# multimodallearning/DG-TTA

Hardware: AMD Instinct MI355X
Metric: TTA-epochs/sec per GPU on 128^3 patch; Dice delta vs reference (higher is better)
Workload: dtype fp16

## Files before the change

### dg_tta_amd/csrc/common.h

```cpp
#pragma once
#include <hip/hip_runtime.h>
#include <hip/hip_bf16.h>
#include <hip/hip_fp16.h>
#include <stdint.h>
#include <stdio.h>
#include <stdarg.h>

#include "../../include/dgtta.h"

#define WAVE 64

#include <atomic>

void dgtta_set_error(const char *fmt, ...);

struct DgttaSwitches {
  int conv_rows, conv_s2, dgrad_s2_allcls, wgrad_tr, wgrad_tr8, wgrad_s2_onepass, convt_wgrad_onepass;
  int convt_gemm, rows_order, in_nt, wgrad_upw, wgrad_xcd, in_gstats, softdice16, conv_ring, wgrad_ring, ha_mfma, wgrad_f32_split, feature_head_mfma, headwarp_mfma, wgrad_flat, wgrad_reduce_taps;
};
const DgttaSwitches &dgtta_switches();

struct DynLdsOnce {
  std::atomic<unsigned long long> mask{0};
};
static inline hipError_t ensure_dyn_lds(DynLdsOnce &o, const void *fn, int bytes) {
  int dev = 0;
  (void)hipGetDevice(&dev);
  const unsigned long long bit = 1ull << (dev & 63);
  if (o.mask.load(std::memory_order_acquire) & bit) return hipSuccess;
  const hipError_t e = hipFuncSetAttribute(fn, hipFuncAttributeMaxDynamicSharedMemorySize, bytes);
  if (e == hipSuccess) o.mask.fetch_or(bit, std::memory_order_release);
  return e;
}

struct RowsGstCtx {
  const void *y;
  long long ldy;
  const float *mr, *gamma, *beta;
  float slope;
  double *out;
  int produced;
// ... 180 lines not shown
```

### dg_tta_amd/csrc/conv_mfma.hip

```cpp
#include "conv_common.h"
#include <stdlib.h>
#include <type_traits>

namespace {

template <typename T, int MBW, int MBH, int MBD, int S, int NB, int KSPC, int NW = 4, bool AC = false>
__global__ __launch_bounds__(NW * 64) void conv3_mfma_kernel(const T *__restrict__ x, View xv, const T *__restrict__ w,
                                                         ConvClasses cs, const float *__restrict__ bias,
                                                         T *__restrict__ y, View yv, int Cin, int Cout, int CinP,
                                                         int CoutP, int tilesW, int tilesH, int tilesD,
                                                         double *__restrict__ stats, int ntaps_src) {
  const int cls = blockIdx.z;
  x += cs.xoff[cls];
  if (!AC) y += cs.yoff[cls];
  const Taps &taps = cs.taps[cls];
  const int accumulate = cs.acc[cls];
  const int Di = xv.D, Hi = xv.H, Wi = xv.W, Do = yv.D, Ho = yv.H, Wo = yv.W;
  typedef ConvCfg<T, MBW, MBH, MBD, S, NB, KSPC> Cfg;
  typedef typename Cfg::G G;
  constexpr int EPV = Cfg::EPV, NG = Cfg::NG, CK = Cfg::CK, NC = Cfg::NC, NV = G::NV, MPW = G::MB / NW, NT = NW * 64;
  extern __shared__ __attribute__((aligned(16))) unsigned char smem[];
  uint4 *sA = reinterpret_cast<uint4 *>(smem);
  uint4 *sB = reinterpret_cast<uint4 *>(smem + Cfg::A_BYTES);

// ... 288 lines not shown
    }
    if (blockIdx.x == 0 && blockIdx.y == 0 && tid == 0) reinterpret_cast<long long *>(stats)[0] = tiles_per_b;
  }
}

template <typename T, int MBW, int MBH, int MBD, int S, int NB, int KSPC, int NW = 4, bool AC = false>
int launch_conv(const ConvLaunch &L, const ConvClasses &cs) {
  typedef ConvCfg<T, MBW, MBH, MBD, S, NB, KSPC> Cfg;
  typedef typename Cfg::G G;
  auto kern = conv3_mfma_kernel<T, MBW, MBH, MBD, S, NB, KSPC, NW, AC>;
  static DynLdsOnce lds_once;
  DG_REQUIRE(ensure_dyn_lds(lds_once, reinterpret_cast<const void *>(kern), (int)Cfg::LDS_BYTES) == hipSuccess,
             DGTTA_ERR_LAUNCH, "conv3_mfma: cannot raise the dynamic LDS limit to %zu", (size_t)Cfg::LDS_BYTES);
  const int tW = cdiv(L.yv.W, G::TW), tH = cdiv(L.yv.H, G::TH), tD = cdiv(L.yv.D, G::TD);
  const int64_t tiles = (int64_t)tW * tH * tD * L.B;
  DG_REQUIRE(tiles < (1ll << 31), DGTTA_ERR_UNSUPPORTED, "conv3_mfma: too many tiles");
  dim3 grid((unsigned)tiles, (unsigned)cdiv(L.CoutP, Cfg::NC), AC ? 1u : (unsigned)cs.n);
  hipLaunchKernelGGL(kern, grid, dim3(NW * 64), Cfg::LDS_BYTES, L.st, (const T *)L.x, L.xv, (const T *)L.w, cs, L.bias, (T *)L.y,
                     L.yv, L.Cin, L.Cout, L.CinP, L.CoutP, tW, tH, tD, L.stats, L.ntaps_src);
  DG_CHECK_LAUNCH(AC ? "conv3_mfma_kernel<all classes>" : "conv3_mfma_kernel");
  return DGTTA_OK;
}

template <typename T>
int dispatch_conv_classes(const ConvLaunch &L, const ConvClasses &cs, int stride) {
  const View &yv = L.yv;
  const bool ring_only = L.xkh || L.dry;
  const long long vox = (long long)yv.D * yv.H * yv.W * L.B;
  if (ring_only && stride != 1) return DGTTA_ERR_UNSUPPORTED;
  if (stride == 0) {
    if (yv.W >= 32) return launch_conv<T, 32, 4, 4, 0, 1, 1, 8>(L, cs);
    if (yv.W >= 16) return launch_conv<T, 16, 4, 4, 0, 1, 1, 8>(L, cs);
    if (vox <= 4096) return launch_conv<T, 8, 2, 2, 0, 1, 1>(L, cs);
    return launch_conv<T, 8, 2, 8, 0, 1, 1, 8>(L, cs);
  }
  if (stride == 1 && sizeof(T) == 2 && yv.W >= 32 && cs.n == 1 && cs.acc[0] == 0 && cs.kseg == 0 && cs.xoff[0] == 0 &&
      cs.yoff[0] == 0) {
    const int rows = dgtta_switches().conv_rows;
    const int is_f16 = (int)std::is_same<T, f16_t>::value;
    bool all_taps = true;
    for (int t = 0; t < 27; ++t) all_taps = all_taps && cs.taps[0].wt[t] >= 0;
    const bool vec_out = L.Cout % 8 == 0 && ((uintptr_t)L.y & 15) == 0 && yv.sw % 8 == 0 && yv.sh % 8 == 0 &&
                         yv.sd % 8 == 0 && yv.sb % 8 == 0;
    const long long njobs = (long long)cdiv(yv.W, 32) * cdiv(yv.H, 8) * cdiv(yv.D, 4) * cdiv(L.CoutP, 32) * L.B;
    if (all_taps && vec_out && ((L.Cin == 32 && L.CinP == 32) || (L.Cin == 64 && L.CinP == 64)) &&
        (njobs >= 512 || dgtta_switches().conv_ring == '1') && dgtta_switches().conv_ring != '0' && rows != '1') {
      const int rc = conv3_ring_launch(L, cs.taps[0], conv3_mfma_max_tiles(yv.D, yv.H, yv.W), is_f16);
      if (rc != DGTTA_ERR_UNSUPPORTED || ring_only) return rc;
    }
    if (ring_only) return DGTTA_ERR_UNSUPPORTED;
    if (all_taps && vec_out && (njobs >= 256 || rows == '1') && rows != '0') return conv3_rows_launch(L, cs.taps[0], is_f16);
  }
  if (ring_only) return DGTTA_ERR_UNSUPPORTED;
  if (stride == 1) {
    if (yv.W >= 32) return launch_conv<T, 32, 4, 4, 1, 1, 1, 8>(L, cs);
    const bool k2 = L.CinP % (4 * Elem<T>::EPV) == 0;
    if (yv.W >= 16) return launch_conv<T, 16, 4, 4, 1, 1, 1, 8>(L, cs);
    if (vox <= 4096 && k2) return launch_conv<T, 8, 2, 2, 1, 1, 2>(L, cs);
    if (vox <= 4096) return launch_conv<T, 8, 2, 2, 1, 1, 1>(L, cs);
    return launch_conv<T, 8, 2, 8, 1, 1, 1, 8>(L, cs);
  }
  if (stride == 2) {
    if (dgtta_switches().conv_s2 == '4') {
      if (yv.W >= 16) return launch_conv<T, 16, 2, 4, 2, 1, 1>(L, cs);
      return launch_conv<T, 8, 2, 4, 2, 1, 1>(L, cs);
    }
    if (dgtta_switches().conv_s2 != '1' && yv.W >= 32 && L.CoutP % 64 == 0) return launch_conv<T, 32, 4, 2, 2, 2, 1, 8>(L, cs);
    if (yv.W >= 32) return launch_conv<T, 32, 4, 2, 2, 1, 1, 8>(L, cs);
    if (yv.W >= 16) return launch_conv<T, 16, 2, 4, 2, 1, 1, 8>(L, cs);
    return launch_conv<T, 8, 2, 4, 2, 1, 1, 8>(L, cs);
  }
  return DGTTA_ERR_UNSUPPORTED;
}

template <typename T>
int dispatch_conv(const ConvLaunch &L, const Taps &taps, int stride, int accumulate) {
  return dispatch_conv_classes<T>(L, single_class(taps, accumulate), stride);
}

template <typename T>
int dgrad_s2_allcls(const ConvLaunch &L, const ConvClasses &cs) {
  if (L.yv.W >= 32) return launch_conv<T, 32, 4, 2, 1, 1, 1, 8, true>(L, cs);
  if (L.yv.W >= 16) return launch_conv<T, 16, 2, 4, 1, 1, 1, 8, true>(L, cs);
  return launch_conv<T, 8, 2, 4, 1, 1, 1, 8, true>(L, cs);
}

template <typename T>
__global__ void conva_pack_kernel(const float *__restrict__ w, T *__restrict__ imgF, T *__restrict__ imgB, int Cin, int Cout,
                                  int CinP, int CoutP, int ntaps) {
  constexpr int EPV = Elem<T>::EPV;
  const int CoutN = (CoutP + 31) / 32 * 32, CinN = (CinP + 31) / 32 * 32;
// ... 11 lines not shown
    }
  }
}

}

int64_t conv3_mfma_max_tiles(int Do, int Ho, int Wo) {
  const int shapes[6][3] = {{4, 4, 32}, {4, 8, 16}, {2, 8, 8}, {8, 8, 8}, {4, 4, 16}, {4, 8, 8}};
  int64_t best = 0;
  for (auto &t : shapes) {
    int64_t n = (int64_t)cdiv(Do, t[0]) * cdiv(Ho, t[1]) * cdiv(Wo, t[2]);
    best = n > best ? n : best;
  }
  return best;
}

int conv3_fwd_mfma(const ConvProblem &P, Src x, const void *w_kmajor, int mirror, const float *bias, Dst y, double *stats,
                   RowsGstCtx *gst) {
  const int stride = P.sd, dtype = P.dtype;
  if ((x.kh || P.dry) && (stride != 1 || dtype == DGTTA_F32)) return DGTTA_ERR_UNSUPPORTED;
  const int Do = P.Do(), Ho = P.Ho(), Wo = P.Wo();
  const ConvLaunch L{x.p, dense_view(P.B, P.Di, P.Hi, P.Wi, x.ld), w_kmajor, bias, y.p, dense_view(P.B, Do, Ho, Wo, y.ld), P.B, P.Cin,
                     P.Cout, P.CinP, P.CoutP, stats, 27, P.st, gst, x.kh, P.dry};
  if (stride == 2 && !mirror && dtype != DGTTA_F32 && dgtta_switches().conv_s2 != '1' && dgtta_switches().conv_s2 != '4') {
    const int rc = conv3_s2_regs(L, conv3_mfma_max_tiles(Do, Ho, Wo), dtype);
    if (rc != DGTTA_ERR_UNSUPPORTED) return rc;
  }
  if (!dtype_ok(dtype) || !operand_ok(epv_of(dtype), x.p, x.kh ? 2 * x.ld : x.ld, P.Cin, P.CinP)) return DGTTA_ERR_UNSUPPORTED;
  DISPATCH_T(dtype, return dispatch_conv<T>(L, identity_taps(mirror), stride, 0));
}

int conv3_dgrad_s2_mfma(const ConvProblem &P, Src dy, const void *w_kmajor, Dst dx, int accumulate) {
  if (!dtype_ok(P.dtype) || !operand_ok(epv_of(P.dtype), dy.p, dy.ld, P.Cout, P.CoutP)) return DGTTA_ERR_UNSUPPORTED;
  View yv;
  const ConvClasses cs = dgrad_parity_classes(P, dx.ld, accumulate, &yv);
  const ConvProblem G = dgrad_as_fwd(P);
  const ConvLaunch L{dy.p, dense_view(P.B, P.Do(), P.Ho(), P.Wo(), dy.ld), w_kmajor, nullptr, dx.p, yv, G.B, G.Cin, G.Cout, G.CinP, G.CoutP,
                     nullptr, 27, P.st};
  const bool allcls = dgtta_switches().dgrad_s2_allcls != '0' && P.CinP % 8 == 0;
  DISPATCH_T(P.dtype, return allcls ? dgrad_s2_allcls<T>(L, cs) : dispatch_conv_classes<T>(L, cs, 1));
}

size_t convT_packed_bytes(int CinP, int CoutP, int dtype) {
  return (size_t)8 * (CinP * n32(CoutP) + CoutP * n32(CinP)) * esize(dtype);
}
size_t conv_image_bytes(int CinP, int CoutP, int dtype) {
  return (size_t)27 * (CinP * n32(CoutP) + CoutP * n32(CinP)) * esize(dtype);
// ... 86 lines not shown
```

### dg_tta_amd/csrc/conv_wgrad.hip

```cpp
#include "conv_wgrad_common.h"

WgradPlan wgrad_plan(int B, int Cin, int Cout, int D, int H, int W, int ncls, int tileW, int tileH) {
  WgradPlan p;
  p.tW = cdiv(W, tileW);
  p.tH = cdiv(H, tileH);
  p.cibs = cdiv(Cin, 32);
  p.cobs = cdiv(Cout, 32);
  const int64_t base = (int64_t)B * p.tW * p.tH * p.cibs * p.cobs * ncls;
  int want = (int)cdiv64(512, base > 0 ? base : 1);
  int maxsplit = D / 4 > 0 ? D / 4 : 1;
  p.nsd = want < 1 ? 1 : (want > maxsplit ? maxsplit : want);
  p.DR = cdiv(D, p.nsd);
  p.nsd = cdiv(D, p.DR);
  p.units = (int64_t)B * p.tW * p.tH * p.nsd;
  return p;
}

size_t conv3_wgrad_mfma_ws_bytes(int B, int Cin, int Cout, int D, int H, int W) {
  WgradPlan p1 = wgrad_plan(B, Cin, Cout, D, H, W, 1, 32, WT::TH), p8 = wgrad_plan(B, Cin, Cout, D, H, W, 8, 32, WT::TH),
            p2 = wgrad_plan(B, Cin, Cout, D, H, W, 1, WT2::TWO, WT2::TH);
  const size_t a = wgrad_slab_bytes(p1, 1), b = wgrad_slab_bytes(p8, 8), c = wgrad_slab_bytes(p2, 1);
  return a > b ? (a > c ? a : c) : (b > c ? b : c);
}

static int units_per_workgroup(int64_t units, int64_t gy, int slots) {
  const int sw = dgtta_switches().wgrad_upw;
  if (sw == '1') return 1;
  if (sw >= '2' && sw <= '4') return (int)(units < sw - '0' ? units : sw - '0');
  int64_t u = units * gy / slots;
  if (u > 4) u = 4;
  if (u > units) u = units;
  return u < 1 ? 1 : (int)u;
}

int wgrad_launch_classes(const WgradLaunch &L, const WgradOut &out, const WgradClasses &wc, const RealTaps &reals) {
  if (!dtype_ok(L.dtype)) return DGTTA_ERR_UNSUPPORTED;
  const int esz = (int)esize(L.dtype), EPV = 16 / esz;
  const View &xv = L.xv, &yv = L.yv;
  if (L.Cout % EPV || xv.sw % EPV || yv.sw % EPV || ((uintptr_t)L.x & 15) || ((uintptr_t)L.dy & 15) ||
      xv.sw < (L.xkh ? 32 : (L.Cin + EPV - 1) / EPV * EPV))
    return DGTTA_ERR_UNSUPPORTED;
  for (int c = 0; c < wc.n; ++c)
    if ((wc.xoff[c] * (long long)esz) % 16 || (wc.yoff[c] * (long long)esz) % 16) return DGTTA_ERR_UNSUPPORTED;
  const DgttaSwitches &sw = dgtta_switches();
  if (L.xkh && (esz != 2 || sw.wgrad_tr == '0' || sw.wgrad_ring == '0')) return DGTTA_ERR_UNSUPPORTED;
  WgradPlan p = wgrad_plan(L.B, L.Cin, L.Cout, yv.D, yv.H, yv.W, wc.n, 32, WT::TH);
  if (L.ws_bytes < wgrad_slab_bytes(p, wc.n) || p.units >= (1ll << 31) || p.cibs * p.cobs > 65535) return DGTTA_ERR_UNSUPPORTED;
  int64_t nslab = p.units;
  int rc = DGTTA_OK;
  if (esz == 2 && sw.wgrad_tr != '0') {
    const bool plain = wc.n == 1 && wc.mask[0] == 0x7ffffffu && wc.xoff[0] == 0 && wc.yoff[0] == 0;
    int64_t g = 0;
    if (plain && !L.xkh && !L.split_leg && sw.wgrad_flat != '0') {
// ... 12 lines not shown
      const int upw = units_per_workgroup(p.units, (int64_t)p.cibs * ((p.cobs + 1) / 2), 256);
      nslab = cdiv64(p.units, upw);
      rc = conv3_wgrad_tr8_launch(L, p, upw, nslab);
    } else {
      const int upw = plain ? units_per_workgroup(p.units, (int64_t)p.cibs * p.cobs, 512) : 1;
      nslab = cdiv64(p.units, upw);
      rc = conv3_wgrad_tr_launch(L, p, wc, plain, upw, nslab);
    }
  } else {
    rc = conv3_wgrad_mfma_launch(L, p, wc);
  }
  if (rc != DGTTA_OK) return rc;
  return wgrad_reduce_launch(L, out, p, wc.n, nslab, reals);
}

static int wgrad_conv(const ConvProblem &P, const WgradLaunch &L, const WgradOut &out) {
  RealTaps reals;
  if (P.sd == 1) return wgrad_launch_classes(L, out, wgrad_single_class(0x7ffffffu, identity_taps(0), &reals), reals);
  if (L.xkh) return DGTTA_ERR_UNSUPPORTED;
  if (L.dtype != DGTTA_F32) {
    const int one = dgtta_switches().wgrad_s2_onepass;
    WgradPlan p = wgrad_plan(L.B, L.Cin, L.Cout, L.yv.D, L.yv.H, L.yv.W, 1, WT2::TWO, WT2::TH);
    if (wgrad_onepass_ok(L, p) && one != '0') {
      const int rc = conv3_wgrad_s2_launch(L, p, p.cobs % 2 == 0 && L.Cout % 64 == 0 && one != '1');
      if (rc != DGTTA_OK) return rc;
      reals.t[0] = identity_taps(0);
      return wgrad_reduce_launch(L, out, p, 1, p.units, reals);
    }
  }
  WgradLaunch C = L;
  const WgradClasses wc = wgrad_parity_classes(P, (int)L.xv.sw, &reals, &C.xv);
  return wgrad_launch_classes(C, out, wc, reals);
}

namespace {
__device__ __forceinline__ void split3(float v, bf16_t &a0, bf16_t &a1, bf16_t &a2) {
  a0 = f32_to_bf16(v);
  const float r1 = v - bf16_to_f32(a0);
  a1 = f32_to_bf16(r1);
  const float r2 = r1 - bf16_to_f32(a1);
  a2 = f32_to_bf16(r2);
}

__global__ __launch_bounds__(256) void split3_bf16_kernel(const float *__restrict__ x, int ld, int C, int lds, int64_t n,
                                                        bf16_t *__restrict__ p0, bf16_t *__restrict__ p1,
                                                        bf16_t *__restrict__ p2) {
  const int groups = lds >> 3;
  const int64_t total = n * groups;
  const bool vec = (ld & 3) == 0 && (C & 7) == 0 && (((uintptr_t)x) & 15) == 0;
  for (int64_t i = (int64_t)blockIdx.x * blockDim.x + threadIdx.x; i < total; i += (int64_t)gridDim.x * blockDim.x) {
// ... 120 lines not shown
```

### dg_tta_amd/csrc/conv_wgrad_common.h

```cpp
#pragma once
#include "conv_common.h"
#include <functional>
#include <type_traits>

namespace dgconv {
struct WgradClasses {
  int n;
  unsigned mask[8];
  long long xoff[8], yoff[8];
};
struct RealTaps {
  Taps t[8];
};
struct WgradPlan {
  int tW, tH, nsd, DR, cibs, cobs;
  int64_t units;
};

struct WgradLaunch {
  const void *x;
  View xv;
  const void *dy;
  View yv;
  int B, Cin, Cout, dtype;
// ... 19 lines not shown
  return (size_t)ncls * p.units * p.cibs * p.cobs * 27 * 1024 * sizeof(float);
}
static inline bool wgrad_onepass_ok(const WgradLaunch &L, const WgradPlan &p) {
  return L.Cout % 8 == 0 && L.xv.sw % 8 == 0 && L.yv.sw % 8 == 0 && !((uintptr_t)L.x & 15) && !((uintptr_t)L.dy & 15) &&
         L.xv.sw >= (L.Cin + 7) / 8 * 8 && L.ws_bytes >= wgrad_slab_bytes(p, 1) && p.units < (1ll << 31) && p.cibs * p.cobs <= 65535;
}

WgradPlan wgrad_plan(int B, int Cin, int Cout, int D, int H, int W, int ncls, int tileW, int tileH);
size_t wgrad_classes_bytes(int B, int Cin, int Cout, int D, int H, int W, int ncls);
int wgrad_launch_classes(const WgradLaunch &L, const WgradOut &out, const WgradClasses &wc, const RealTaps &reals);
size_t wgrad_split_plane_bytes(int B, int C, int D, int H, int W);
typedef std::function<int(const bf16_t *x, int ldx, const bf16_t *dy, int lddy, int accumulate)> WgradSplitLeg;
int wgrad_f32_split(const SplitOperand &x, const SplitOperand &dy, void *ws, size_t ws_bytes, size_t slab_bytes, int accumulate,
                    hipStream_t st, const WgradSplitLeg &leg);

int conv3_wgrad_ring_launch(const WgradLaunch &L, int *rc);

int conv3_wgrad_mfma_launch(const WgradLaunch &L, const WgradPlan &p, const WgradClasses &wc);
int conv3_wgrad_tr_launch(const WgradLaunch &L, const WgradPlan &p, const WgradClasses &wc, bool plain, int upw, int64_t nslab);
int conv3_wgrad_tr8_launch(const WgradLaunch &L, const WgradPlan &p, int upw, int64_t nslab);

int64_t wgrad_flat_launch(const WgradLaunch &L, int *rc);

int conv3_wgrad_s2_launch(const WgradLaunch &L, const WgradPlan &p, bool two_blocks);

int wgrad_reduce_launch(const WgradLaunch &L, const WgradOut &out, const WgradPlan &p, int ncls, int64_t nslab, const RealTaps &reals);

namespace {

inline WgradClasses wgrad_single_class(unsigned tapmask, const Taps &real, RealTaps *reals) {
  WgradClasses wc{};
  wc.n = 1;
  wc.mask[0] = tapmask;
  reals->t[0] = real;
  return wc;
}

inline WgradClasses wgrad_parity_classes(const ConvProblem &P, int ldx, RealTaps *reals, View *xv) {
  const int ks[3] = {P.kd, 3, 3}, ss[3] = {P.sd, P.sh, P.sw};
  WgradClasses wc{};
  *xv = dense_view(1, P.Di, P.Hi, P.Wi, ldx);
  for (int c = 0; c < P.noff(); ++c) {
    const Parity par = class_parity(c, P.sd, P.sh, P.sw);
    unsigned mask = 0;
    Taps rt;
    for (int t = 0; t < 27; ++t) {
      const int u[3] = {t / 9 - 1, (t / 3) % 3 - 1, t % 3 - 1};
// ... 112 lines not shown
```

### dg_tta_amd/csrc/conv_wgrad_s2.hip

```cpp
#include "conv_wgrad_common.h"

namespace {

template <typename T16 = bf16_t>
__global__ __launch_bounds__(256, 2) void conv3_wgrad_tr_s2_kernel(const bf16_t *__restrict__ x, View xv,
                                                                   const bf16_t *__restrict__ dy, View yv,
                                                                   float *__restrict__ slabs, int Cin, int Cout, int tilesW,
                                                                   int tilesH, int nsd, int DR, int cobs) {
  const int D = yv.D, H = yv.H, W = yv.W;
  extern __shared__ __attribute__((aligned(16))) unsigned char smem[];
  unsigned char *sX = smem;
  unsigned char *sY = smem + WT2::NXS * WT2::X_SLICE_B;
  const int tid = threadIdx.x, lane = tid & 63;
  const int wave = __builtin_amdgcn_readfirstlane(tid >> 6);

  int t = xcd_unit(1);
  const int tw = t % tilesW;
  t /= tilesW;
  const int th = t % tilesH;
  t /= tilesH;
  const int ds = t % nsd;
  const int b = t / nsd;
  const int cib = blockIdx.y / cobs, cob = blockIdx.y % cobs;
  const int h0 = th * WT2::TH, w0 = tw * WT2::TWO;
  const int d_begin = ds * DR, d_end = (d_begin + DR < D) ? d_begin + DR : D;
  const bf16_t *xb = x + b * xv.sb + cib * 32;
  const bf16_t *yb = dy + b * yv.sb + cob * 32;
  const int cin_lim = (Cin + 7) / 8 * 8;
  const int l_vox = lane >> 2, l_chunk = lane & 3;

  auto xslot = [&](int xd) { return (xd + WT2::NXS) % WT2::NXS; };
  auto issue_x_slice = [&](int xd, int i) __attribute__((always_inline)) {
    const int idx = wave + 4 * i;
    if (idx >= WT2::NPX1) return;
    const int r = idx / 3, pi = idx % 3;
    if (pi == 2 && lane >= 4) return;
    const int gh = 2 * h0 - 1 + r, wx = 16 * pi + l_vox, gw = 2 * w0 - 1 + wx;
    const bool ok = (unsigned)xd < (unsigned)xv.D && (unsigned)gh < (unsigned)xv.H && (unsigned)gw < (unsigned)xv.W &&
                    cib * 32 + l_chunk * 8 < cin_lim;
    const void *src = ok ? (const void *)(xb + xd * xv.sd + gh * xv.sh + gw * xv.sw + l_chunk * 8) : (const void *)&g_zero16;
    dma16_to_lds(src, lds_addr_of(sX + xslot(xd) * WT2::X_SLICE_B + r * WT2::X_ROW_B + pi * 1024));
  };
  auto issue_y_slice = [&](int yd) __attribute__((always_inline)) {
    if (wave >= WT2::TH) return;
    const int gh = h0 + wave, gw = w0 + l_vox;
    const bool ok = (unsigned)yd < (unsigned)D && gh < H && gw < W && cob * 32 + l_chunk * 8 < Cout;
    const void *src = ok ? (const void *)(yb + yd * yv.sd + gh * yv.sh + gw * yv.sw + l_chunk * 8) : (const void *)&g_zero16;
    dma16_to_lds(src, lds_addr_of(sY + (yd & 1) * WT2::Y_SLICE_B + wave * WT2::Y_ROW_B));
  };
  constexpr int NPXW = (WT2::NPX1 + 3) / 4;

  const int kq = (lane >> 5) * 8 + ((lane & 15) >> 2), cpart = ((lane >> 4) & 1) * 32 + (lane & 3) * 8;
  const int lane_off_y = kq * 64 + cpart, lane_off_x = kq * 128 + cpart;

  int tap_kd[7], tap_off[7];
#pragma unroll
  for (int i = 0; i < 7; ++i) {
    const int tc = wave + 4 * i < 27 ? wave + 4 * i : 26;
    tap_kd[i] = tc / 9;
    tap_off[i] = ((tc / 3) % 3) * WT2::X_ROW_B + (tc % 3) * 64;
  }
  f32x16_t acc[7];
#pragma unroll
  for (int i = 0; i < 7; ++i)
#pragma unroll
    for (int q = 0; q < 16; ++q) acc[i][q] = 0.f;

#pragma unroll
  for (int sl = -1; sl <= 1; ++sl)
#pragma unroll
    for (int i = 0; i < NPXW; ++i) issue_x_slice(2 * d_begin + sl, i);
  issue_y_slice(d_begin);
  dma_wait_all();
  lds_barrier();

  for (int d = d_begin; d < d_end; ++d) {
    if (d + 1 < d_end) {
#pragma unroll
      for (int i = 0; i < NPXW; ++i) issue_x_slice(2 * d + 2, i);
#pragma unroll
      for (int i = 0; i < NPXW; ++i) issue_x_slice(2 * d + 3, i);
      issue_y_slice(d + 1);
    }
    const unsigned char *ys = sY + (d & 1) * WT2::Y_SLICE_B + lane_off_y;
    int slice_off[3];
#pragma unroll
    for (int kd = 0; kd < 3; ++kd) slice_off[kd] = xslot(2 * d + kd - 1) * WT2::X_SLICE_B;
    int so_t[7];
#pragma unroll
    for (int i = 0; i < 7; ++i) so_t[i] = (tap_kd[i] == 0 ? slice_off[0] : (tap_kd[i] == 1 ? slice_off[1] : slice_off[2])) + tap_off[i];
#pragma unroll
    for (int oh = 0; oh < WT2::TH; ++oh) {
      const s16x4_t blo = __builtin_amdgcn_ds_read_tr16_b64_v4i16((lds_s16x4_t *)(ys + oh * WT2::Y_ROW_B));
      const s16x4_t bhi = __builtin_amdgcn_ds_read_tr16_b64_v4i16((lds_s16x4_t *)(ys + oh * WT2::Y_ROW_B + 4 * 64));
      const s16x8_t bv = {blo[0], blo[1], blo[2], blo[3], bhi[0], bhi[1], bhi[2], bhi[3]};
      const bf16x8_t bfr = __builtin_bit_cast(bf16x8_t, bv);
      bf16x8_t afr[7];
#pragma unroll
      for (int i = 0; i < 7; ++i) {
        const unsigned char *pa = sX + lane_off_x + so_t[i] + 2 * oh * WT2::X_ROW_B;
        const s16x4_t alo = __builtin_amdgcn_ds_read_tr16_b64_v4i16((lds_s16x4_t *)pa);
        const s16x4_t ahi = __builtin_amdgcn_ds_read_tr16_b64_v4i16((lds_s16x4_t *)(pa + 4 * 128));
        const s16x8_t av = {alo[0], alo[1], alo[2], alo[3], ahi[0], ahi[1], ahi[2], ahi[3]};
        afr[i] = __builtin_bit_cast(bf16x8_t, av);
      }
#pragma unroll
      for (int i = 0; i < 7; ++i) acc[i] = mfma32_tr<T16>(afr[i], bfr, acc[i]);
    }
    dma_wait_all();
    lds_barrier();
  }

  float *slab = slabs + ((int64_t)blockIdx.y * gridDim.x + blockIdx.x) * (27 * 1024);
  const int co = lane & 31, hh = lane >> 5;
#pragma unroll
  for (int i = 0; i < 7; ++i) {
    const int tap = wave + 4 * i;
    if (tap < 27) {
#pragma unroll
      for (int q = 0; q < 16; ++q) slab[(tap * 32 + (q & 3) + 8 * (q >> 2) + 4 * hh) * 32 + co] = acc[i][q];
    }
  }
}

struct WT2X {
  static constexpr int NCO = 2, LA = 2;
  static constexpr int NXS = 3 + 2 * LA, NYS = LA + 1;
  static constexpr int Y_STEP_B = NCO * WT2::Y_SLICE_B;
  static constexpr int LDS_BYTES = NXS * WT2::X_SLICE_B + NYS * Y_STEP_B;
};

template <typename T16 = bf16_t>
__global__ __launch_bounds__(512, 2) void conv3_wgrad_tr_s2x_kernel(const bf16_t *__restrict__ x, View xv,
                                                                    const bf16_t *__restrict__ dy, View yv,
                                                                    float *__restrict__ slabs, int Cin, int Cout, int tilesW,
                                                                    int tilesH, int nsd, int DR, int cobs) {
  const int D = yv.D, H = yv.H, W = yv.W;
  extern __shared__ __attribute__((aligned(16))) unsigned char smem[];
  unsigned char *sX = smem;
  unsigned char *sY = smem + WT2X::NXS * WT2::X_SLICE_B;
  const int tid = threadIdx.x, lane = tid & 63;
  const int wave = __builtin_amdgcn_readfirstlane(tid >> 6);
  const int tg = wave & 3, cb = wave >> 2;

  int t = xcd_unit(1);
  const int tw = t % tilesW;
  t /= tilesW;
  const int th = t % tilesH;
  t /= tilesH;
  const int ds = t % nsd;
  const int b = t / nsd;
  const int cogs = cobs / 2;
  const int cib = blockIdx.y / cogs, cog = blockIdx.y % cogs;
  const int h0 = th * WT2::TH, w0 = tw * WT2::TWO;
  const int d_begin = ds * DR, d_end = (d_begin + DR < D) ? d_begin + DR : D;
  const bf16_t *xb = x + b * xv.sb + cib * 32;
  const bf16_t *yb = dy + b * yv.sb + cog * 64;
  const int cin_lim = (Cin + 7) / 8 * 8;
  const int l_vox = lane >> 2, l_chunk = lane & 3;

  auto xslot = [&](int xd) { return (xd + WT2X::NXS) % WT2X::NXS; };
  auto issue_x_slice = [&](int xd) __attribute__((always_inline)) {
#pragma unroll
    for (int i = 0; i < 2; ++i) {
      int idx = wave + 8 * i;
      idx = idx < WT2::NPX1 ? idx : WT2::NPX1 - 1;
      const int r = idx / 3, pi = idx % 3;
      const int gh = 2 * h0 - 1 + r, wx = 16 * pi + l_vox, gw = 2 * w0 - 1 + wx;
      const bool ok = (unsigned)xd < (unsigned)xv.D && (unsigned)gh < (unsigned)xv.H && (unsigned)gw < (unsigned)xv.W &&
                      cib * 32 + l_chunk * 8 < cin_lim && (pi < 2 || lane < 4);
      const void *src = ok ? (const void *)(xb + xd * xv.sd + gh * xv.sh + gw * xv.sw + l_chunk * 8) : (const void *)&g_zero16;
      if (pi < 2 || lane < 12)
        dma16_to_lds(src, lds_addr_of(sX + xslot(xd) * WT2::X_SLICE_B + r * WT2::X_ROW_B + pi * 1024));
    }
  };
  auto issue_y_slice = [&](int yd) __attribute__((always_inline)) {
    const int row = wave & 1, blk = (wave >> 1) & 1;
    const int gh = h0 + row, gw = w0 + l_vox;
    const bool ok = (unsigned)yd < (unsigned)D && gh < H && gw < W && cog * 64 + blk * 32 + l_chunk * 8 < Cout;
    const void *src = ok ? (const void *)(yb + yd * yv.sd + gh * yv.sh + gw * yv.sw + blk * 32 + l_chunk * 8)
// ... 2 lines not shown
  };
  auto issue_step = [&](int od) __attribute__((always_inline)) {
    issue_x_slice(2 * od);
    issue_x_slice(2 * od + 1);
    issue_y_slice(od);
  };

  const int kq = (lane >> 5) * 8 + ((lane & 15) >> 2), cpart = ((lane >> 4) & 1) * 32 + (lane & 3) * 8;
  const int lane_off_y = kq * 64 + cpart, lane_off_x = kq * 128 + cpart;

  int tap_kd[7], tap_off[7];
#pragma unroll
  for (int i = 0; i < 7; ++i) {
    const int tc = tg + 4 * i < 27 ? tg + 4 * i : 26;
    tap_kd[i] = tc / 9;
    tap_off[i] = ((tc / 3) % 3) * WT2::X_ROW_B + (tc % 3) * 64;
  }
  f32x16_t acc[7];
#pragma unroll
  for (int i = 0; i < 7; ++i)
#pragma unroll
    for (int q = 0; q < 16; ++q) acc[i][q] = 0.f;

  issue_x_slice(2 * d_begin - 1);
  issue_step(d_begin);
  if (d_begin + 1 < d_end) issue_step(d_begin + 1);
  dma_wait_all();
  lds_barrier();

  for (int d = d_begin; d < d_end; ++d) {
    const bool ahead = d + WT2X::LA < d_end;
    if (ahead) issue_step(d + WT2X::LA);
    const unsigned char *ys = sY + (d % WT2X::NYS) * WT2X::Y_STEP_B + cb * WT2::Y_SLICE_B + lane_off_y;
    int slice_off[3];
#pragma unroll
    for (int kd = 0; kd < 3; ++kd) slice_off[kd] = xslot(2 * d + kd - 1) * WT2::X_SLICE_B;
    int so_t[7];
#pragma unroll
    for (int i = 0; i < 7; ++i) so_t[i] = (tap_kd[i] == 0 ? slice_off[0] : (tap_kd[i] == 1 ? slice_off[1] : slice_off[2])) + tap_off[i];
#pragma unroll
    for (int oh = 0; oh < WT2::TH; ++oh) {
      const s16x4_t blo = __builtin_amdgcn_ds_read_tr16_b64_v4i16((lds_s16x4_t *)(ys + oh * WT2::Y_ROW_B));
      const s16x4_t bhi = __builtin_amdgcn_ds_read_tr16_b64_v4i16((lds_s16x4_t *)(ys + oh * WT2::Y_ROW_B + 4 * 64));
      const s16x8_t bv = {blo[0], blo[1], blo[2], blo[3], bhi[0], bhi[1], bhi[2], bhi[3]};
      const bf16x8_t bfr = __builtin_bit_cast(bf16x8_t, bv);
      bf16x8_t afr[7];
#pragma unroll
      for (int i = 0; i < 7; ++i) {
        const unsigned char *pa = sX + lane_off_x + so_t[i] + 2 * oh * WT2::X_ROW_B;
        const s16x4_t alo = __builtin_amdgcn_ds_read_tr16_b64_v4i16((lds_s16x4_t *)pa);
        const s16x4_t ahi = __builtin_amdgcn_ds_read_tr16_b64_v4i16((lds_s16x4_t *)(pa + 4 * 128));
        const s16x8_t av = {alo[0], alo[1], alo[2], alo[3], ahi[0], ahi[1], ahi[2], ahi[3]};
        afr[i] = __builtin_bit_cast(bf16x8_t, av);
      }
#pragma unroll
      for (int i = 0; i < 7; ++i) acc[i] = mfma32_tr<T16>(afr[i], bfr, acc[i]);
    }
    if (ahead) asm volatile("s_waitcnt vmcnt(5)" ::: "memory");
    else dma_wait_all();
    lds_barrier();
  }

  const int pair = cib * cobs + cog * 2 + cb;
  float *slab = slabs + ((int64_t)pair * gridDim.x + blockIdx.x) * (27 * 1024);
  const int co = lane & 31, hh = lane >> 5;
#pragma unroll
  for (int i = 0; i < 7; ++i) {
    const int tap = tg + 4 * i;
    if (tap < 27) {
#pragma unroll
      for (int q = 0; q < 16; ++q) slab[(tap * 32 + (q & 3) + 8 * (q >> 2) + 4 * hh) * 32 + co] = acc[i][q];
    }
  }
}

template <typename T16>
int s2_launch(const WgradLaunch &L, const WgradPlan &p, bool two_blocks) {
  static DynLdsOnce once, once_x;
  if (two_blocks) {
    DG_REQUIRE(ensure_dyn_lds(once_x, reinterpret_cast<const void *>(conv3_wgrad_tr_s2x_kernel<T16>), (int)WT2X::LDS_BYTES) ==
                   hipSuccess, DGTTA_ERR_LAUNCH, "wgrad_tr_s2x: cannot raise the dynamic LDS limit");
    hipLaunchKernelGGL(conv3_wgrad_tr_s2x_kernel<T16>, dim3((unsigned)p.units, (unsigned)(p.cibs * (p.cobs / 2))), dim3(512),
                       WT2X::LDS_BYTES, L.st, (const bf16_t *)L.x, L.xv, (const bf16_t *)L.dy, L.yv, (float *)L.ws, L.Cin, L.Cout, p.tW,
                       p.tH, p.nsd, p.DR, p.cobs);
  } else {
    DG_REQUIRE(ensure_dyn_lds(once, reinterpret_cast<const void *>(conv3_wgrad_tr_s2_kernel<T16>), (int)WT2::LDS_BYTES) ==
                   hipSuccess, DGTTA_ERR_LAUNCH, "wgrad_tr_s2: cannot raise the dynamic LDS limit");
    hipLaunchKernelGGL(conv3_wgrad_tr_s2_kernel<T16>, dim3((unsigned)p.units, (unsigned)(p.cibs * p.cobs)), dim3(256),
                       WT2::LDS_BYTES, L.st, (const bf16_t *)L.x, L.xv, (const bf16_t *)L.dy, L.yv, (float *)L.ws, L.Cin, L.Cout, p.tW,
                       p.tH, p.nsd, p.DR, p.cobs);
  }
  DG_CHECK_LAUNCH("conv3_wgrad_tr_s2_kernel");
  return DGTTA_OK;
}

}

int conv3_wgrad_s2_launch(const WgradLaunch &L, const WgradPlan &p, bool two_blocks) {
  return L.dtype == DGTTA_F16 ? s2_launch<f16_t>(L, p, two_blocks) : s2_launch<bf16_t>(L, p, two_blocks);
}
```

### dg_tta_amd/csrc/lib.hip

```cpp
#include "common.h"
#include <string.h>

static thread_local char g_err[512] = "";

void dgtta_set_error(const char *fmt, ...) {
  va_list ap;
  va_start(ap, fmt);
  vsnprintf(g_err, sizeof(g_err), fmt, ap);
  va_end(ap);
}

extern "C" int dgtta_version(void) { return 60200;  }
extern "C" const char *dgtta_last_error(void) { return g_err; }

#include <mutex>
#include <stdlib.h>

static std::atomic<const DgttaSwitches *> g_switches{nullptr};
static std::once_flag g_switches_once;


static int env_char(const char *name) {
  const char *v = getenv(name);
  return (v && v[0] && !v[1] && v[0] >= '0' && v[0] <= '9') ? (int)(unsigned char)v[0] : -1;
// ... 4 lines not shown
  s->conv_rows = env_char("DGTTA_CONV_ROWS");
  s->conv_s2 = env_char("DGTTA_CONV_S2");
  s->convt_gemm = env_char("DGTTA_CONVT_GEMM");
  s->rows_order = env_char("DGTTA_ROWS_ORDER");
  s->wgrad_upw = env_char("DGTTA_WGRAD_UPW");
  s->wgrad_xcd = env_char("DGTTA_WGRAD_XCD");
  s->in_nt = env_char("DGTTA_IN_NT");
  s->in_nt = s->in_nt == '0' ? '0' : '1';
  s->dgrad_s2_allcls = env_char("DGTTA_DGRAD_S2_ALLCLS");
  s->wgrad_tr = env_char("DGTTA_WGRAD_TR");
  s->wgrad_tr8 = env_char("DGTTA_WGRAD_TR8");
  s->wgrad_s2_onepass = env_char("DGTTA_WGRAD_S2_ONEPASS");
  s->convt_wgrad_onepass = env_char("DGTTA_CONVT_WGRAD_ONEPASS");
  s->in_gstats = env_char("DGTTA_IN_GSTATS");
  s->softdice16 = env_char("DGTTA_SOFTDICE16");
  s->conv_ring = env_char("DGTTA_CONV_RING");
  s->wgrad_ring = env_char("DGTTA_WGRAD_RING");
  s->ha_mfma = env_char("DGTTA_HA_MFMA");
  s->wgrad_f32_split = env_char("DGTTA_WGRAD_F32_SPLIT");
  s->feature_head_mfma = env_char("DGTTA_FEATURE_HEAD_MFMA");
  s->headwarp_mfma = env_char("DGTTA_HEADWARP_MFMA");
  s->wgrad_flat = env_char("DGTTA_WGRAD_FLAT");
  s->wgrad_reduce_taps = env_char("DGTTA_WGRAD_REDUCE_TAPS");
  if (s->conv_ring != '0' && s->conv_ring != '1' && s->conv_ring != '3') s->conv_ring = -1;
  if (s->wgrad_ring != '0' && s->wgrad_ring != '1' && s->wgrad_ring != '4' && s->wgrad_ring != '5' && s->wgrad_ring != '6') s->wgrad_ring = -1;
  if (s->convt_gemm != '0' && s->convt_gemm != '1') s->convt_gemm = -1;
  return s;
}

const DgttaSwitches &dgtta_switches() {
  std::call_once(g_switches_once, [] { g_switches.store(read_switches(), std::memory_order_release); });
  return *g_switches.load(std::memory_order_acquire);
}

extern "C" int dgtta_reload_env(void) {
  (void)dgtta_switches();
  g_switches.store(read_switches(), std::memory_order_release);
  return DGTTA_OK;
}
```

Baseline: 6.602.

## Loop multiple units per workgroup in stride-2 wgrad; add two-block conv variant

The stride-2 weight-gradient kernels now process several spatial units per workgroup, looping over them and accumulating into one slab. This shrinks the grid and the number of partial slabs the reduction kernel must sum. A heuristic picks up to 8 units per workgroup from the occupancy slots. Separately, the small-width stride-2 forward conv can pick a variant with two Cout blocks when enough workgroups exist. Batching units trades parallelism for less reduction traffic and may leave CUs idle on small grids.

```diff
diff --git a/dg_tta_amd/csrc/common.h b/dg_tta_amd/csrc/common.h
--- a/dg_tta_amd/csrc/common.h
+++ b/dg_tta_amd/csrc/common.h
@@ -16,7 +16,7 @@
 
 struct DgttaSwitches {
   int conv_rows, conv_s2, dgrad_s2_allcls, wgrad_tr, wgrad_tr8, wgrad_s2_onepass, convt_wgrad_onepass;
-  int convt_gemm, rows_order, in_nt, wgrad_upw, wgrad_xcd, in_gstats, softdice16, conv_ring, wgrad_ring, ha_mfma, wgrad_f32_split, feature_head_mfma, headwarp_mfma, wgrad_flat, wgrad_reduce_taps;
+  int convt_gemm, rows_order, in_nt, wgrad_upw, wgrad_xcd, in_gstats, softdice16, conv_ring, wgrad_ring, ha_mfma, wgrad_f32_split, feature_head_mfma, headwarp_mfma, wgrad_flat, wgrad_reduce_taps, wgrad_s2_upw, conv_s2_nb;
 };
 const DgttaSwitches &dgtta_switches();
 
diff --git a/dg_tta_amd/csrc/conv_mfma.hip b/dg_tta_amd/csrc/conv_mfma.hip
--- a/dg_tta_amd/csrc/conv_mfma.hip
+++ b/dg_tta_amd/csrc/conv_mfma.hip
@@ -334,6 +334,14 @@
   return DGTTA_OK;
 }
 
+static bool s2_two_blocks(const ConvLaunch &L, int ncls, int tw) {
+  const int sw = dgtta_switches().conv_s2_nb;
+  if (sw == '1') return false;
+  if (sw == '2' || sw == '4') return true;
+  const long long wgs = (long long)cdiv(L.yv.W, tw) * cdiv(L.yv.H, 64 / tw) * cdiv(L.yv.D, 4) * L.B * (L.CoutP / 64) * ncls;
+  return wgs >= 256;
+}
+
 template <typename T>
 int dispatch_conv_classes(const ConvLaunch &L, const ConvClasses &cs, int stride) {
   const View &yv = L.yv;
@@ -379,6 +387,10 @@
     }
     if (dgtta_switches().conv_s2 != '1' && yv.W >= 32 && L.CoutP % 64 == 0) return launch_conv<T, 32, 4, 2, 2, 2, 1, 8>(L, cs);
     if (yv.W >= 32) return launch_conv<T, 32, 4, 2, 2, 1, 1, 8>(L, cs);
+    if constexpr (sizeof(T) == 2) {
+      if (L.CoutP % 64 == 0 && s2_two_blocks(L, cs.n, yv.W >= 16 ? 16 : 8))
+        return yv.W >= 16 ? launch_conv<T, 16, 2, 4, 2, 2, 1, 8>(L, cs) : launch_conv<T, 8, 2, 4, 2, 2, 1, 8>(L, cs);
+    }
     if (yv.W >= 16) return launch_conv<T, 16, 2, 4, 2, 1, 1, 8>(L, cs);
     return launch_conv<T, 8, 2, 4, 2, 1, 1, 8>(L, cs);
   }
@@ -436,7 +448,8 @@
   const int Do = P.Do(), Ho = P.Ho(), Wo = P.Wo();
   const ConvLaunch L{x.p, dense_view(P.B, P.Di, P.Hi, P.Wi, x.ld), w_kmajor, bias, y.p, dense_view(P.B, Do, Ho, Wo, y.ld), P.B, P.Cin,
                      P.Cout, P.CinP, P.CoutP, stats, 27, P.st, gst, x.kh, P.dry};
-  if (stride == 2 && !mirror && dtype != DGTTA_F32 && dgtta_switches().conv_s2 != '1' && dgtta_switches().conv_s2 != '4') {
+  const int s2sw = dgtta_switches().conv_s2;
+  if (stride == 2 && !mirror && dtype != DGTTA_F32 && s2sw != '1' && s2sw != '2' && s2sw != '4') {
     const int rc = conv3_s2_regs(L, conv3_mfma_max_tiles(Do, Ho, Wo), dtype);
     if (rc != DGTTA_ERR_UNSUPPORTED) return rc;
   }
diff --git a/dg_tta_amd/csrc/conv_wgrad.hip b/dg_tta_amd/csrc/conv_wgrad.hip
--- a/dg_tta_amd/csrc/conv_wgrad.hip
+++ b/dg_tta_amd/csrc/conv_wgrad.hip
@@ -23,12 +23,11 @@
   return a > b ? (a > c ? a : c) : (b > c ? b : c);
 }
 
-static int units_per_workgroup(int64_t units, int64_t gy, int slots) {
-  const int sw = dgtta_switches().wgrad_upw;
+static int units_per_workgroup(int64_t units, int64_t gy, int slots, int sw = dgtta_switches().wgrad_upw, int cap = 4) {
   if (sw == '1') return 1;
-  if (sw >= '2' && sw <= '4') return (int)(units < sw - '0' ? units : sw - '0');
+  if (sw >= '2' && sw <= '0' + cap) return (int)(units < sw - '0' ? units : sw - '0');
   int64_t u = units * gy / slots;
-  if (u > 4) u = 4;
+  if (u > cap) u = cap;
   if (u > units) u = units;
   return u < 1 ? 1 : (int)u;
 }
@@ -87,10 +86,13 @@
     const int one = dgtta_switches().wgrad_s2_onepass;
     WgradPlan p = wgrad_plan(L.B, L.Cin, L.Cout, L.yv.D, L.yv.H, L.yv.W, 1, WT2::TWO, WT2::TH);
     if (wgrad_onepass_ok(L, p) && one != '0') {
-      const int rc = conv3_wgrad_s2_launch(L, p, p.cobs % 2 == 0 && L.Cout % 64 == 0 && one != '1');
+      const bool two = p.cobs % 2 == 0 && L.Cout % 64 == 0 && one != '1';
+      const int upw = L.split_leg ? 1 : units_per_workgroup(p.units, (int64_t)p.cibs * (two ? p.cobs / 2 : p.cobs), two ? 256 : 512,
+                                                            dgtta_switches().wgrad_s2_upw, 8);
+      const int rc = conv3_wgrad_s2_launch(L, p, two, upw);
       if (rc != DGTTA_OK) return rc;
       reals.t[0] = identity_taps(0);
-      return wgrad_reduce_launch(L, out, p, 1, p.units, reals);
+      return wgrad_reduce_launch(L, out, p, 1, cdiv64(p.units, upw), reals);
     }
   }
   WgradLaunch C = L;
diff --git a/dg_tta_amd/csrc/conv_wgrad_common.h b/dg_tta_amd/csrc/conv_wgrad_common.h
--- a/dg_tta_amd/csrc/conv_wgrad_common.h
+++ b/dg_tta_amd/csrc/conv_wgrad_common.h
@@ -65,7 +65,7 @@
 
 int64_t wgrad_flat_launch(const WgradLaunch &L, int *rc);
 
-int conv3_wgrad_s2_launch(const WgradLaunch &L, const WgradPlan &p, bool two_blocks);
+int conv3_wgrad_s2_launch(const WgradLaunch &L, const WgradPlan &p, bool two_blocks, int upw);
 
 int wgrad_reduce_launch(const WgradLaunch &L, const WgradOut &out, const WgradPlan &p, int ncls, int64_t nslab, const RealTaps &reals);
 
diff --git a/dg_tta_amd/csrc/conv_wgrad_s2.hip b/dg_tta_amd/csrc/conv_wgrad_s2.hip
--- a/dg_tta_amd/csrc/conv_wgrad_s2.hip
+++ b/dg_tta_amd/csrc/conv_wgrad_s2.hip
@@ -6,7 +6,7 @@
 __global__ __launch_bounds__(256, 2) void conv3_wgrad_tr_s2_kernel(const bf16_t *__restrict__ x, View xv,
                                                                    const bf16_t *__restrict__ dy, View yv,
                                                                    float *__restrict__ slabs, int Cin, int Cout, int tilesW,
-                                                                   int tilesH, int nsd, int DR, int cobs) {
+                                                                   int tilesH, int nsd, int DR, int cobs, int units, int upw) {
   const int D = yv.D, H = yv.H, W = yv.W;
   extern __shared__ __attribute__((aligned(16))) unsigned char smem[];
   unsigned char *sX = smem;
@@ -14,18 +14,21 @@
   const int tid = threadIdx.x, lane = tid & 63;
   const int wave = __builtin_amdgcn_readfirstlane(tid >> 6);
 
-  int t = xcd_unit(1);
-  const int tw = t % tilesW;
-  t /= tilesW;
-  const int th = t % tilesH;
-  t /= tilesH;
-  const int ds = t % nsd;
-  const int b = t / nsd;
+  const int u_begin = xcd_unit(1) * upw, u_end = u_begin + upw < units ? u_begin + upw : units;
   const int cib = blockIdx.y / cobs, cob = blockIdx.y % cobs;
-  const int h0 = th * WT2::TH, w0 = tw * WT2::TWO;
-  const int d_begin = ds * DR, d_end = (d_begin + DR < D) ? d_begin + DR : D;
-  const bf16_t *xb = x + b * xv.sb + cib * 32;
-  const bf16_t *yb = dy + b * yv.sb + cob * 32;
+  int h0, w0, d_begin, d_end;
+  const bf16_t *xb, *yb;
+  auto enter_unit = [&](int t) __attribute__((always_inline)) {
+    const int tw = t % tilesW;
+    t /= tilesW;
+    const int th = t % tilesH;
+    t /= tilesH;
+    const int ds = t % nsd, b = t / nsd;
+    h0 = th * WT2::TH, w0 = tw * WT2::TWO;
+    d_begin = ds * DR, d_end = (d_begin + DR < D) ? d_begin + DR : D;
+    xb = x + b * xv.sb + cib * 32;
+    yb = dy + b * yv.sb + cob * 32;
+  };
   const int cin_lim = (Cin + 7) / 8 * 8;
   const int l_vox = lane >> 2, l_chunk = lane & 3;
 
@@ -66,49 +69,52 @@
 #pragma unroll
     for (int q = 0; q < 16; ++q) acc[i][q] = 0.f;
 
-#pragma unroll
-  for (int sl = -1; sl <= 1; ++sl)
-#pragma unroll
-    for (int i = 0; i < NPXW; ++i) issue_x_slice(2 * d_begin + sl, i);
-  issue_y_slice(d_begin);
-  dma_wait_all();
-  lds_barrier();
-
-  for (int d = d_begin; d < d_end; ++d) {
-    if (d + 1 < d_end) {
-#pragma unroll
-      for (int i = 0; i < NPXW; ++i) issue_x_slice(2 * d + 2, i);
-#pragma unroll
-      for (int i = 0; i < NPXW; ++i) issue_x_slice(2 * d + 3, i);
-      issue_y_slice(d + 1);
-    }
-    const unsigned char *ys = sY + (d & 1) * WT2::Y_SLICE_B + lane_off_y;
-    int slice_off[3];
-#pragma unroll
-    for (int kd = 0; kd < 3; ++kd) slice_off[kd] = xslot(2 * d + kd - 1) * WT2::X_SLICE_B;
-    int so_t[7];
-#pragma unroll
-    for (int i = 0; i < 7; ++i) so_t[i] = (tap_kd[i] == 0 ? slice_off[0] : (tap_kd[i] == 1 ? slice_off[1] : slice_off[2])) + tap_off[i];
-#pragma unroll
-    for (int oh = 0; oh < WT2::TH; ++oh) {
-      const s16x4_t blo = __builtin_amdgcn_ds_read_tr16_b64_v4i16((lds_s16x4_t *)(ys + oh * WT2::Y_ROW_B));
-      const s16x4_t bhi = __builtin_amdgcn_ds_read_tr16_b64_v4i16((lds_s16x4_t *)(ys + oh * WT2::Y_ROW_B + 4 * 64));
-      const s16x8_t bv = {blo[0], blo[1], blo[2], blo[3], bhi[0], bhi[1], bhi[2], bhi[3]};
-      const bf16x8_t bfr = __builtin_bit_cast(bf16x8_t, bv);
-      bf16x8_t afr[7];
-#pragma unroll
-      for (int i = 0; i < 7; ++i) {
-        const unsigned char *pa = sX + lane_off_x + so_t[i] + 2 * oh * WT2::X_ROW_B;
-        const s16x4_t alo = __builtin_amdgcn_ds_read_tr16_b64_v4i16((lds_s16x4_t *)pa);
-        const s16x4_t ahi = __builtin_amdgcn_ds_read_tr16_b64_v4i16((lds_s16x4_t *)(pa + 4 * 128));
-        const s16x8_t av = {alo[0], alo[1], alo[2], alo[3], ahi[0], ahi[1], ahi[2], ahi[3]};
-        afr[i] = __builtin_bit_cast(bf16x8_t, av);
-      }
-#pragma unroll
-      for (int i = 0; i < 7; ++i) acc[i] = mfma32_tr<T16>(afr[i], bfr, acc[i]);
-    }
+  for (int u = u_begin; u < u_end; ++u) {
+    enter_unit(u);
+#pragma unroll
+    for (int sl = -1; sl <= 1; ++sl)
+#pragma unroll
+      for (int i = 0; i < NPXW; ++i) issue_x_slice(2 * d_begin + sl, i);
+    issue_y_slice(d_begin);
     dma_wait_all();
     lds_barrier();
+
+    for (int d = d_begin; d < d_end; ++d) {
+      if (d + 1 < d_end) {
+#pragma unroll
+        for (int i = 0; i < NPXW; ++i) issue_x_slice(2 * d + 2, i);
+#pragma unroll
+        for (int i = 0; i < NPXW; ++i) issue_x_slice(2 * d + 3, i);
+        issue_y_slice(d + 1);
+      }
+      const unsigned char *ys = sY + (d & 1) * WT2::Y_SLICE_B + lane_off_y;
+      int slice_off[3];
+#pragma unroll
+      for (int kd = 0; kd < 3; ++kd) slice_off[kd] = xslot(2 * d + kd - 1) * WT2::X_SLICE_B;
+      int so_t[7];
+#pragma unroll
+      for (int i = 0; i < 7; ++i) so_t[i] = (tap_kd[i] == 0 ? slice_off[0] : (tap_kd[i] == 1 ? slice_off[1] : slice_off[2])) + tap_off[i];
+#pragma unroll
+      for (int oh = 0; oh < WT2::TH; ++oh) {
+        const s16x4_t blo = __builtin_amdgcn_ds_read_tr16_b64_v4i16((lds_s16x4_t *)(ys + oh * WT2::Y_ROW_B));
+        const s16x4_t bhi = __builtin_amdgcn_ds_read_tr16_b64_v4i16((lds_s16x4_t *)(ys + oh * WT2::Y_ROW_B + 4 * 64));
+        const s16x8_t bv = {blo[0], blo[1], blo[2], blo[3], bhi[0], bhi[1], bhi[2], bhi[3]};
+        const bf16x8_t bfr = __builtin_bit_cast(bf16x8_t, bv);
+        bf16x8_t afr[7];
+#pragma unroll
+        for (int i = 0; i < 7; ++i) {
+          const unsigned char *pa = sX + lane_off_x + so_t[i] + 2 * oh * WT2::X_ROW_B;
+          const s16x4_t alo = __builtin_amdgcn_ds_read_tr16_b64_v4i16((lds_s16x4_t *)pa);
+          const s16x4_t ahi = __builtin_amdgcn_ds_read_tr16_b64_v4i16((lds_s16x4_t *)(pa + 4 * 128));
+          const s16x8_t av = {alo[0], alo[1], alo[2], alo[3], ahi[0], ahi[1], ahi[2], ahi[3]};
+          afr[i] = __builtin_bit_cast(bf16x8_t, av);
+        }
+#pragma unroll
+        for (int i = 0; i < 7; ++i) acc[i] = mfma32_tr<T16>(afr[i], bfr, acc[i]);
+      }
+      dma_wait_all();
+      lds_barrier();
+    }
   }
 
   float *slab = slabs + ((int64_t)blockIdx.y * gridDim.x + blockIdx.x) * (27 * 1024);
@@ -134,7 +140,7 @@
 __global__ __launch_bounds__(512, 2) void conv3_wgrad_tr_s2x_kernel(const bf16_t *__restrict__ x, View xv,
                                                                     const bf16_t *__restrict__ dy, View yv,
                                                                     float *__restrict__ slabs, int Cin, int Cout, int tilesW,
-                                                                    int tilesH, int nsd, int DR, int cobs) {
+                                                                    int tilesH, int nsd, int DR, int cobs, int units, int upw) {
   const int D = yv.D, H = yv.H, W = yv.W;
   extern __shared__ __attribute__((aligned(16))) unsigned char smem[];
   unsigned char *sX = smem;
@@ -143,19 +149,22 @@
   const int wave = __builtin_amdgcn_readfirstlane(tid >> 6);
   const int tg = wave & 3, cb = wave >> 2;
 
-  int t = xcd_unit(1);
-  const int tw = t % tilesW;
-  t /= tilesW;
-  const int th = t % tilesH;
-  t /= tilesH;
-  const int ds = t % nsd;
-  const int b = t / nsd;
+  const int u_begin = xcd_unit(1) * upw, u_end = u_begin + upw < units ? u_begin + upw : units;
   const int cogs = cobs / 2;
   const int cib = blockIdx.y / cogs, cog = blockIdx.y % cogs;
-  const int h0 = th * WT2::TH, w0 = tw * WT2::TWO;
-  const int d_begin = ds * DR, d_end = (d_begin + DR < D) ? d_begin + DR : D;
-  const bf16_t *xb = x + b * xv.sb + cib * 32;
-  const bf16_t *yb = dy + b * yv.sb + cog * 64;
+  int h0, w0, d_begin, d_end;
+  const bf16_t *xb, *yb;
+  auto enter_unit = [&](int t) __attribute__((always_inline)) {
+    const int tw = t % tilesW;
+    t /= tilesW;
+    const int th = t % tilesH;
+    t /= tilesH;
+    const int ds = t % nsd, b = t / nsd;
+    h0 = th * WT2::TH, w0 = tw * WT2::TWO;
+    d_begin = ds * DR, d_end = (d_begin + DR < D) ? d_begin + DR : D;
+    xb = x + b * xv.sb + cib * 32;
+    yb = dy + b * yv.sb + cog * 64;
+  };
   const int cin_lim = (Cin + 7) / 8 * 8;
   const int l_vox = lane >> 2, l_chunk = lane & 3;
 
@@ -204,43 +213,46 @@
 #pragma unroll
     for (int q = 0; q < 16; ++q) acc[i][q] = 0.f;
 
-  issue_x_slice(2 * d_begin - 1);
-  issue_step(d_begin);
-  if (d_begin + 1 < d_end) issue_step(d_begin + 1);
-  dma_wait_all();
-  lds_barrier();
-
-  for (int d = d_begin; d < d_end; ++d) {
-    const bool ahead = d + WT2X::LA < d_end;
-    if (ahead) issue_step(d + WT2X::LA);
-    const unsigned char *ys = sY + (d % WT2X::NYS) * WT2X::Y_STEP_B + cb * WT2::Y_SLICE_B + lane_off_y;
-    int slice_off[3];
-#pragma unroll
-    for (int kd = 0; kd < 3; ++kd) slice_off[kd] = xslot(2 * d + kd - 1) * WT2::X_SLICE_B;
-    int so_t[7];
-#pragma unroll
-    for (int i = 0; i < 7; ++i) so_t[i] = (tap_kd[i] == 0 ? slice_off[0] : (tap_kd[i] == 1 ? slice_off[1] : slice_off[2])) + tap_off[i];
-#pragma unroll
-    for (int oh = 0; oh < WT2::TH; ++oh) {
-      const s16x4_t blo = __builtin_amdgcn_ds_read_tr16_b64_v4i16((lds_s16x4_t *)(ys + oh * WT2::Y_ROW_B));
-      const s16x4_t bhi = __builtin_amdgcn_ds_read_tr16_b64_v4i16((lds_s16x4_t *)(ys + oh * WT2::Y_ROW_B + 4 * 64));
-      const s16x8_t bv = {blo[0], blo[1], blo[2], blo[3], bhi[0], bhi[1], bhi[2], bhi[3]};
-      const bf16x8_t bfr = __builtin_bit_cast(bf16x8_t, bv);
-      bf16x8_t afr[7];
-#pragma unroll
-      for (int i = 0; i < 7; ++i) {
-        const unsigned char *pa = sX + lane_off_x + so_t[i] + 2 * oh * WT2::X_ROW_B;
-        const s16x4_t alo = __builtin_amdgcn_ds_read_tr16_b64_v4i16((lds_s16x4_t *)pa);
-        const s16x4_t ahi = __builtin_amdgcn_ds_read_tr16_b64_v4i16((lds_s16x4_t *)(pa + 4 * 128));
-        const s16x8_t av = {alo[0], alo[1], alo[2], alo[3], ahi[0], ahi[1], ahi[2], ahi[3]};
-        afr[i] = __builtin_bit_cast(bf16x8_t, av);
+  for (int u = u_begin; u < u_end; ++u) {
+    enter_unit(u);
+    issue_x_slice(2 * d_begin - 1);
+    issue_step(d_begin);
+    if (d_begin + 1 < d_end) issue_step(d_begin + 1);
+    dma_wait_all();
+    lds_barrier();
+
+    for (int d = d_begin; d < d_end; ++d) {
+      const bool ahead = d + WT2X::LA < d_end;
+      if (ahead) issue_step(d + WT2X::LA);
+      const unsigned char *ys = sY + (d % WT2X::NYS) * WT2X::Y_STEP_B + cb * WT2::Y_SLICE_B + lane_off_y;
+      int slice_off[3];
+#pragma unroll
+      for (int kd = 0; kd < 3; ++kd) slice_off[kd] = xslot(2 * d + kd - 1) * WT2::X_SLICE_B;
+      int so_t[7];
+#pragma unroll
+      for (int i = 0; i < 7; ++i) so_t[i] = (tap_kd[i] == 0 ? slice_off[0] : (tap_kd[i] == 1 ? slice_off[1] : slice_off[2])) + tap_off[i];
+#pragma unroll
+      for (int oh = 0; oh < WT2::TH; ++oh) {
+        const s16x4_t blo = __builtin_amdgcn_ds_read_tr16_b64_v4i16((lds_s16x4_t *)(ys + oh * WT2::Y_ROW_B));
+        const s16x4_t bhi = __builtin_amdgcn_ds_read_tr16_b64_v4i16((lds_s16x4_t *)(ys + oh * WT2::Y_ROW_B + 4 * 64));
+        const s16x8_t bv = {blo[0], blo[1], blo[2], blo[3], bhi[0], bhi[1], bhi[2], bhi[3]};
+        const bf16x8_t bfr = __builtin_bit_cast(bf16x8_t, bv);
+        bf16x8_t afr[7];
+#pragma unroll
+        for (int i = 0; i < 7; ++i) {
+          const unsigned char *pa = sX + lane_off_x + so_t[i] + 2 * oh * WT2::X_ROW_B;
+          const s16x4_t alo = __builtin_amdgcn_ds_read_tr16_b64_v4i16((lds_s16x4_t *)pa);
+          const s16x4_t ahi = __builtin_amdgcn_ds_read_tr16_b64_v4i16((lds_s16x4_t *)(pa + 4 * 128));
+          const s16x8_t av = {alo[0], alo[1], alo[2], alo[3], ahi[0], ahi[1], ahi[2], ahi[3]};
+          afr[i] = __builtin_bit_cast(bf16x8_t, av);
+        }
+#pragma unroll
+        for (int i = 0; i < 7; ++i) acc[i] = mfma32_tr<T16>(afr[i], bfr, acc[i]);
       }
-#pragma unroll
-      for (int i = 0; i < 7; ++i) acc[i] = mfma32_tr<T16>(afr[i], bfr, acc[i]);
-    }
-    if (ahead) asm volatile("s_waitcnt vmcnt(5)" ::: "memory");
-    else dma_wait_all();
-    lds_barrier();
+      if (ahead) asm volatile("s_waitcnt vmcnt(5)" ::: "memory");
+      else dma_wait_all();
+      lds_barrier();
+    }
   }
 
   const int pair = cib * cobs + cog * 2 + cb;
@@ -257,20 +269,21 @@
 }
 
 template <typename T16>
-int s2_launch(const WgradLaunch &L, const WgradPlan &p, bool two_blocks) {
+int s2_launch(const WgradLaunch &L, const WgradPlan &p, bool two_blocks, int upw) {
+  const unsigned nslab = (unsigned)cdiv64(p.units, upw);
   static DynLdsOnce once, once_x;
   if (two_blocks) {
     DG_REQUIRE(ensure_dyn_lds(once_x, reinterpret_cast<const void *>(conv3_wgrad_tr_s2x_kernel<T16>), (int)WT2X::LDS_BYTES) ==
                    hipSuccess, DGTTA_ERR_LAUNCH, "wgrad_tr_s2x: cannot raise the dynamic LDS limit");
-    hipLaunchKernelGGL(conv3_wgrad_tr_s2x_kernel<T16>, dim3((unsigned)p.units, (unsigned)(p.cibs * (p.cobs / 2))), dim3(512),
+    hipLaunchKernelGGL(conv3_wgrad_tr_s2x_kernel<T16>, dim3(nslab, (unsigned)(p.cibs * (p.cobs / 2))), dim3(512),
                        WT2X::LDS_BYTES, L.st, (const bf16_t *)L.x, L.xv, (const bf16_t *)L.dy, L.yv, (float *)L.ws, L.Cin, L.Cout, p.tW,
-                       p.tH, p.nsd, p.DR, p.cobs);
+                       p.tH, p.nsd, p.DR, p.cobs, (int)p.units, upw);
   } else {
     DG_REQUIRE(ensure_dyn_lds(once, reinterpret_cast<const void *>(conv3_wgrad_tr_s2_kernel<T16>), (int)WT2::LDS_BYTES) ==
                    hipSuccess, DGTTA_ERR_LAUNCH, "wgrad_tr_s2: cannot raise the dynamic LDS limit");
-    hipLaunchKernelGGL(conv3_wgrad_tr_s2_kernel<T16>, dim3((unsigned)p.units, (unsigned)(p.cibs * p.cobs)), dim3(256),
+    hipLaunchKernelGGL(conv3_wgrad_tr_s2_kernel<T16>, dim3(nslab, (unsigned)(p.cibs * p.cobs)), dim3(256),
                        WT2::LDS_BYTES, L.st, (const bf16_t *)L.x, L.xv, (const bf16_t *)L.dy, L.yv, (float *)L.ws, L.Cin, L.Cout, p.tW,
-                       p.tH, p.nsd, p.DR, p.cobs);
+                       p.tH, p.nsd, p.DR, p.cobs, (int)p.units, upw);
   }
   DG_CHECK_LAUNCH("conv3_wgrad_tr_s2_kernel");
   return DGTTA_OK;
@@ -278,6 +291,6 @@
 
 }
 
-int conv3_wgrad_s2_launch(const WgradLaunch &L, const WgradPlan &p, bool two_blocks) {
-  return L.dtype == DGTTA_F16 ? s2_launch<f16_t>(L, p, two_blocks) : s2_launch<bf16_t>(L, p, two_blocks);
-}
+int conv3_wgrad_s2_launch(const WgradLaunch &L, const WgradPlan &p, bool two_blocks, int upw) {
+  return L.dtype == DGTTA_F16 ? s2_launch<f16_t>(L, p, two_blocks, upw) : s2_launch<bf16_t>(L, p, two_blocks, upw);
+}
diff --git a/dg_tta_amd/csrc/lib.hip b/dg_tta_amd/csrc/lib.hip
--- a/dg_tta_amd/csrc/lib.hip
+++ b/dg_tta_amd/csrc/lib.hip
@@ -50,6 +50,8 @@
   s->headwarp_mfma = env_char("DGTTA_HEADWARP_MFMA");
   s->wgrad_flat = env_char("DGTTA_WGRAD_FLAT");
   s->wgrad_reduce_taps = env_char("DGTTA_WGRAD_REDUCE_TAPS");
+  s->wgrad_s2_upw = env_char("DGTTA_WGRAD_S2_UPW");
+  s->conv_s2_nb = env_char("DGTTA_CONV_S2_NB");
   if (s->conv_ring != '0' && s->conv_ring != '1' && s->conv_ring != '3') s->conv_ring = -1;
   if (s->wgrad_ring != '0' && s->wgrad_ring != '1' && s->wgrad_ring != '4' && s->wgrad_ring != '5' && s->wgrad_ring != '6') s->wgrad_ring = -1;
   if (s->convt_gemm != '0' && s->convt_gemm != '1') s->convt_gemm = -1;
```

Result: no change. 6.612 (median of 3 runs) (+0.1%).
